# kubernetes-sigs/kube-batch

Measured on AMD Instinct MI355X. Metric: pod-node scoring evals/sec + binds/sec, 100k tasks x 10k nodes snapshot, higher is better.
Workload: dtype f64+i64

## Files before the change

### kube-batch_amd/csrc/kb_commit_sel.hip

```cpp
#include <string.h>

#include <algorithm>

#include "kb_k9.hpp"
#include "kb_repair.hpp"

#define K9S_PREP0 5u
#define K9S_PREPS 3u
#define K9S_SPIN_LIMIT (1u << 21)

__device__ __forceinline__ uint32_t k9s_ld(const uint32_t *p) { return __hip_atomic_load(p, __ATOMIC_ACQUIRE, __HIP_MEMORY_SCOPE_WORKGROUP); }
__device__ __forceinline__ void k9s_st(uint32_t *p, uint32_t v) { __hip_atomic_store(p, v, __ATOMIC_RELEASE, __HIP_MEMORY_SCOPE_WORKGROUP); }
__device__ __forceinline__ bool k9s_wait(K9Sync &Y, const uint32_t *p, uint32_t need, uint32_t nap = 1u) {
  uint32_t spins = 0;
  for (;;) {
    if (k9s_ld(p) >= need) return true;
    if ((++spins & 31u) == 0u) {
      if (k9s_ld(&Y.stop) | k9s_ld(&Y.err)) return k9s_ld(p) >= need;
      if (spins > K9S_SPIN_LIMIT) { k9s_st(&Y.err, 1u); return false; }
    }
    if (nap == 0u) { } else if (nap == 1u) __builtin_amdgcn_s_sleep(1); else if (nap <= 4u) __builtin_amdgcn_s_sleep(4); else __builtin_amdgcn_s_sleep(16);
  }
}

__global__ void __launch_bounds__(K9_THREADS) k_commit_select(const K9KernArgs ka) {
  KbCommitArgs a = ka.hot;
  {
    const unsigned char __attribute__((address_space(4))) *kp = (const unsigned char __attribute__((address_space(4))) *)__builtin_amdgcn_kernarg_segment_ptr();
    a.dev = (const KbDev *)(kp + offsetof(K9KernArgs, dev));
    a.round = (const KbRound *)(kp + offsetof(K9KernArgs, round));
  }
  extern __shared__ __align__(16) unsigned char k9_smem[];
  if ((blockIdx.x & 7u) != 0u && a.round->lists_ready != nullptr) {
    const uint32_t row = blockIdx.x - 1u - blockIdx.x / 8u;
    if (row < a.n_mrows && !KB_CHAIN_BROKEN(*a.round)) kb_repair_row<K9_THREADS>(*a.dev, *a.round, k9_smem, row, threadIdx.x);
    return;
  }
  if (k9_preamble(a)) return;
  const uint32_t tid = threadIdx.x, lane = tid & 63, wave = tid >> 6;
  const uint32_t S = a.n_mrows, W = a.n_rows;
  const K9Layout lo = k9_layout(W, S, a.L, a.NP, a.R, true);
  unsigned char *k9_base_ = k9_smem;
  K9_LDS_VIEWS(lo)
  (void)shp; (void)S; (void)dk; (void)ckey; (void)cpos;
  K9Sel &X = *reinterpret_cast<K9Sel *>(k9_smem + lo.sel);
  K9Sync &Y = X.sync;
  const unsigned long long t_start = wall_clock64();
#ifdef KB_K9_TRACE
  unsigned long long t_stage[2] = {0ull, 0ull};
  const bool staged = k9_prologue(a, lo, k9_smem, tid, 0u, t_stage);
#else
  const bool staged = k9_prologue(a, lo, k9_smem, tid, 0u);
#endif
  if (!staged) {
    if (tid == 0) k9_publish_skipped(a);
// ... 18 lines not shown
  __syncthreads();
  if (tid < W) {
    uint32_t w = tid >> 5, mword = X.brk[w] & (0xFFFFFFFFu >> (31u - (tid & 31u)));
    while (mword == 0u) { w--; mword = X.brk[w]; }
    const uint32_t p = 32u * w + (31u - (uint32_t)__clz((int)mword));
    if ((tid - p) % K9_SEL_MAXRUN == 0u) atomicOr(&X.stm[tid >> 5], 1u << (tid & 31));
  }
  __syncthreads();
  if (tid < W && ((X.stm[tid >> 5] >> (tid & 31)) & 1u)) {
    uint32_t kidx = (uint32_t)__popc(X.stm[tid >> 5] & ((1u << (tid & 31)) - 1u));
    for (uint32_t w = 0; w < (tid >> 5); w++) kidx += (uint32_t)__popc(X.stm[w]);
    X.runs[kidx] = (uint16_t)tid;
  }
  __syncthreads();
  uint32_t K = 0;
  for (uint32_t w = 0; w < 8; w++) K += (uint32_t)__popc(X.stm[w]);
  {
    uint4 rr = make_uint4(0u, 0u, 0u, 0u);
    uint32_t i0c = 0u;
    uint32_t rlen = 0u;
    if (tid < K) { i0c = X.runs[tid]; rr = rinfo[i0c]; rlen = ((tid + 1u < K) ? (uint32_t)X.runs[tid + 1u] : W) - i0c; }
    __syncthreads();
    if (tid < K) rinfo[tid] = make_uint4(i0c | (rlen << 16), rr.y, rr.z, rr.w);
    __syncthreads();
  }

#ifdef KB_K9_TRACE
  uint32_t tacc[10] = {0, 0, 0, 0, 0, 0, 0, 0, 0, 0};
  const unsigned long long t_tab = wall_clock64();
  tacc[1] = (uint32_t)(t_stage[0] - t_start); tacc[9] = (uint32_t)(t_stage[1] - t_stage[0]); tacc[2] = (uint32_t)(t_tab - t_stage[1]);
  unsigned long long tlast = __builtin_readcyclecounter();
#define K9S_TR(k, t0) do { if (lane == 0) atomicAdd(&X.tr[k], (uint32_t)(__builtin_readcyclecounter() - (t0))); } while (0)
#define K9S_NOW() __builtin_readcyclecounter()
#else
#define K9S_TR(k, t0) do { (void)(t0); } while (0)
#define K9S_NOW() 0ull
#endif
#ifndef KB_K9_NAP_PREP
#define KB_K9_NAP_PREP 1u
#endif
  constexpr uint32_t nap_prep = KB_K9_NAP_PREP, nap_dk = 1u;
#if !defined(KB_K9_PRIO) || KB_K9_PRIO
#define K9S_SETPRIO(p) __builtin_amdgcn_s_setprio(p)
#else
#define K9S_SETPRIO(p) do { } while (0)
#endif
  const unsigned long long lt = (1ull << lane) - 1ull;
  gptrd gi, gr;
  { const KbDev &d = *a.dev; gi = (gptrd)d.idle; gr = (gptrd)d.rel; }
#define K9S_RUN_HEADER_OF(ri_)                                                                                         \
  const uint32_t hx_ = (uint32_t)__builtin_amdgcn_readfirstlane((int)(ri_).x);                                          \
  const uint32_t i0 = hx_ & 0xFFFFu, r = hx_ >> 16, s = (uint32_t)__builtin_amdgcn_readfirstlane((int)(ri_).y);          \
  const uint32_t fl0 = (uint32_t)__builtin_amdgcn_readfirstlane((int)(ri_).z), km0 = (uint32_t)__builtin_amdgcn_readfirstlane((int)(ri_).w); \
  const bool plain0 = (fl0 & 1u) && (km0 == 0u || (fl0 & 4u));                                                         \
  const bool sel_run = !a.backfill && plain0 && r >= 2u && a.whole;             \
  (void)sel_run; (void)i0;
#define K9S_RUN_SHAPE(kk)                                                                                              \
  const K9Shape sh = shapes[s];                                                                                        \
  const double *si = sinit + (size_t)s * RS;                                                                           \
  const double *rres = rowres + ((kk) % K9S_PREPS) * (uint32_t)a.R;    \
  const double *rqv = plain0 ? si : rres + 2;                                             \
  (void)rqv; (void)rres;
#define K9S_RUN_HEADER(kk)                                                                                             \
  const uint4 ri_ = rinfo[(kk)];                                                                                       \
  K9S_RUN_HEADER_OF(ri_)                                                                                               \
  K9S_RUN_SHAPE(kk)

  if (wave == 0) {
    K9S_SETPRIO(3);
    uint32_t nd = 0, n_dirty_rows = 0, n_runs = 0, n_slow = 0, i_end = 0, reason_end = KB_REASON_DONE;
    uint32_t prev_nd0 = 0, prev_pc = 0;
    bool prev_chg = true;
    bool prev_all = false;
    uint4 hd_next = rinfo[0];
    for (uint32_t k = 0; k < K; k++) {
      uint32_t lane_i = tid;
      asm volatile("" : "+v"(lane_i));
      const uint4 hd = hd_next;
      if (k + 1u < K) hd_next = rinfo[k + 1u];
      K9S_RUN_HEADER_OF(hd)
      K9_STAMP(3);
      {
        uint32_t spins = 0;
        bool ok = true;
        for (;;) {
          const uint32_t *wp = (lane_i == 0u) ? (prev_all ? &Y.seq_spec : &Y.seq_cand) : (prev_chg ? &Y.seq_dk[(lane_i - 1u) & 3u] : &Y.seq_early[(lane_i - 1u) & 3u]);
          const uint32_t v = (lane_i < 5u) ? k9s_ld(wp) : 0xFFFFFFFFu;
          if (__ballot(v < k + 1u) == 0ull) break;
          if ((++spins & 31u) == 0u && (k9s_ld(&Y.err) || spins > K9S_SPIN_LIMIT)) { k9s_st(&Y.err, 1u); ok = false; break; }
          __builtin_amdgcn_s_sleep(1);
        }
        if (!ok) { reason_end = KB_REASON_INTERNAL; i_end = i0; break; }
      }
      if (prev_all && lane_i == 0) k9s_st(&Y.seq_cand, k + 1u);
      const uint32_t ncand = Y.ncand_at[k & 3u];
      const K9Sel::Cand &CD = X.cand[k & 1u];
      const uint32_t *dk = X.dkb[k & 1u];
      uint32_t *chg = Y.chg[k & 1u];
      uint32_t ck = CD.ckey[lane_i], k1 = CD.ck1[lane_i], ckind = CD.ckind[lane_i];
      const uint32_t cpos = CD.cpos[lane_i];
      uint32_t m = (lane_i < 4u) ? (prev_chg ? Y.mdk[k & 1u][lane_i] : Y.mdko[k & 1u][lane_i]) : 0u;
      if (!prev_chg && lane_i >= 4u && lane_i - 4u < prev_pc) m = dk[prev_nd0 + lane_i - 4u];
      if (lane_i < 10u) chg[lane_i] = 0u;
      K9_STAMP(0);
      if (lane_i >= ncand) { ck = 0u; k1 = 0u; ckind = 0u; }
      m = wave_max_u32(m);
      uint32_t pc = 0, j = 0, reason = KB_REASON_DONE, n_dirty = 0, sc_dirty = 0;
      bool chg_any = false;
      bool run_done = false;
      if (!a.backfill && plain0) {
        const uint32_t cmin = (ncand == r) ? rl32(ck, r - 1u) : 0u;
        const unsigned long long deeper = __ballot(lane_i + 1u < r && ckind == 0u && k1 > cmin);
        if (ncand == r && m < cmin && !deeper) {
          const unsigned long long pipes = __ballot(lane_i < r && ckind != 0u);
          const uint32_t n_take = pipes ? (uint32_t)__ffsll((unsigned long long)pipes) : r;
          if (pipes) reason = KB_REASON_PIPELINED;
          if (lane_i < n_take) {
            const uint32_t n = nmaskbits - (ck & nmaskbits);
            ldec[i0 + lane_i] = (unsigned long long)n | ((unsigned long long)ckind << 32);
            atomicOr(&bitmap[n >> 5], 1u << (n & 31));
            if (km0) {
              const double *rqv = sinit + (size_t)s * RS;
              const uint32_t rnm = CD.crnm[lane_i];
              atomicOr(&chg[(nd + lane_i) >> 5], 1u << ((nd + lane_i) & 31));
              const bool has_map = ckind ? (rnm >> 31) : (rnm & 0x7FFFFFFFu);
              if (has_map)
                for (uint32_t mm = km0, dd = 0; mm; mm >>= 1, dd++)
                  if (mm & 1u) k9_sc_sub(ckind ? gr : gi, a.NP, dd, n, rqv[dd]);
            }
          }
          if (km0) { sc_dirty = 1; chg_any = true; }
          pc = n_take; j = n_take;
          run_done = true;
          if (lane_i == 0 && r >= 2u) atomicAdd(&X.stat[0], 1u);
          K9_STAMP(8);
        }
      }
      if (!run_done) {
      K9S_RUN_SHAPE(k)
      uint32_t rnm = 0;
      if (lane_i < ncand) rnm = CD.crnm[lane_i];
      double res0 = sh.init0, res1 = sh.init1;
      if (!plain0) { res0 = rres[0]; res1 = rres[1]; }
      uint32_t d0 = 0u, d1 = 0u, d2 = 0u, d3 = 0u;
      bool have_d = false;
#define K9S_LOAD_D() do { if (!have_d) { d0 = (lane_i < nd) ? dk[lane_i] : 0u; d1 = (lane_i + 64 < nd) ? dk[lane_i + 64] : 0u; d2 = (lane_i + 128 < nd) ? dk[lane_i + 128] : 0u; \
                                        d3 = (lane_i + 192 < nd) ? dk[lane_i + 192] : 0u; have_d = true; } } while (0)
      bool sel_done = false;
      if (sel_run) {
        K9S_LOAD_D();
        bool pooled = false;
        while (j < r) {
          const uint32_t rem = r - j;
          const uint32_t fidx = pc + rem - 1u;
          uint32_t thr = max(fidx < ncand ? rl32(ck, fidx) : 0u, 1u);
          const uint32_t kc = lane_i < pc ? k1 : (lane_i < ncand ? ck : 0u);
          bool isc, is0, is1, is2, is3;
          unsigned long long bc, b0, b1, b2, b3;
          uint32_t nc_, n0_, n1_, n2_, n3_, nC;
          for (uint32_t again = 0;; again++) {
            isc = kc >= thr; is0 = d0 >= thr; is1 = d1 >= thr; is2 = d2 >= thr; is3 = d3 >= thr;
            bc = __ballot(isc); b0 = __ballot(is0);
            nc_ = (uint32_t)__popcll(bc); n0_ = (uint32_t)__popcll(b0);
            b1 = 0ull; b2 = 0ull; b3 = 0ull; n1_ = 0u; n2_ = 0u; n3_ = 0u;
            if (nd > 64u) { b1 = __ballot(is1); n1_ = (uint32_t)__popcll(b1); }
            if (nd > 128u) { b2 = __ballot(is2); b3 = __ballot(is3); n2_ = (uint32_t)__popcll(b2); n3_ = (uint32_t)__popcll(b3); }
            nC = nc_ + n0_ + n1_ + n2_ + n3_;
            if (nC <= 32u || again) break;
            uint32_t lm = max(max(max(d0, d1), max(d2, d3)), kc);
            for (uint32_t t = 0; t < 5u; t++) {
              const uint32_t mx = wave_max_u32(lm);
              if (mx == 0u) break;
              thr = mx;
              if (lm == mx) lm = 0u;
            }
          }
          if (nC == 0u) { reason = KB_REASON_NO_FEASIBLE; break; }
          {
            const uint32_t p_c = (uint32_t)__popcll(bc & lt), p_0 = nc_ + (uint32_t)__popcll(b0 & lt);
            if (isc) { X.c_slot[p_c] = (nd + lane_i) | (lane_i >= pc ? 0x80000000u : 0u); X.c_key[p_c] = kc; }
            if (is0) { X.c_slot[p_0] = lane_i; X.c_key[p_0] = d0; }
// ... 236 lines not shown
          if (bf_bulk) {
            const uint32_t left1 = (uint32_t)(rl64(cur8, F_CLS_LEFT) >> 32);
            bulk = 1u + min(r - j - 1u, left1);
            if (bulk > 1u) {
              if (lane_i == F_NZC) { double z = u2d(cur8); for (uint32_t t = 1; t < bulk; t++) z += sh.nzc; cur8 = d2u(z); }
              else if (lane_i == F_NZM) { double z = u2d(cur8); for (uint32_t t = 1; t < bulk; t++) z += sh.nzm; cur8 = d2u(z); }
              else if (lane_i == F_CLS_LEFT) cur8 -= ((unsigned long long)(bulk - 1u) << 32);
            }
          }
          if (lane_i < K9_NF) st[lane_i] = cur8;
          if (lane_i < bulk) ldec[i0 + j + lane_i] = (unsigned long long)n | ((unsigned long long)kind << 32);
          j += bulk - 1u;
          n_dirty += bulk - 1u;
          K9_WAVE_FENCE();
          const bool more = j + 1u < r && !kind;
          const uint32_t adjm1 = (!kind && has_map) ? km0 : 0u;
          uint32_t nk = 0u;
          if (more) nk = k9_eval_v(a, sh, k9_load(st), scs, gi, gr, si, adjm1, 1.0, rqv, nb, nmaskbits);
          if (km0 && has_map) {
            if (sc_lane && ((km0 >> sd) & 1u)) k9_sc_sub(kind ? gr : gi, a.NP, sd, n, rqv[sd]);
            sc_dirty = 1;
          }
          if (more) {
            if (lane_i == L) {
              if (is_new) k1 = nk;
              else if (wsel == 0) d0 = nk; else if (wsel == 1) d1 = nk; else if (wsel == 2) d2 = nk; else d3 = nk;
            }
            m = wave_max_u32(max(max(max(d0, d1), max(d2, d3)), (lane_i < pc) ? k1 : 0u));
          }
          n_dirty++;
        }
        if (kind) { j++; reason = KB_REASON_PIPELINED; break; }
      }
      }
      if (sc_dirty) __threadfence();
      const uint32_t i_next = i0 + j;
      uint32_t stop = (reason != KB_REASON_DONE || k + 1u >= K) ? 1u : 0u;
      if (!stop && a.has_aff && !a.backfill && i_next != 0u) {
        const uint32_t fln = (uint32_t)__builtin_amdgcn_readfirstlane((int)hd_next.z);
        if (fln & 2u) { reason = KB_REASON_RENORM; stop = 1u; }
      }
      if (pc) { const uint32_t cp = rl32(cpos, pc - 1u); if (lane_i == 0) cursor[s] = cp + 1u; }
      prev_nd0 = nd; prev_pc = pc; prev_all = pc == ncand;
      K9_WAVE_FENCE();
      prev_chg = chg_any;
      nd += pc; n_dirty_rows += n_dirty; n_runs += 1u; n_slow += plain0 ? 0u : 1u;
      i_end = i_next; reason_end = reason;
      if (lane_i == 0) {
        Y.nd_at[(k + 1u) & 3u] = nd;
        Y.spec_ok[(k + 1u) & 3u] = prev_all ? 1u : 0u;
        if (stop) k9s_st(&Y.stop, 1u);
        k9s_st(&Y.seq_done, k + 1u);
      }
      if (stop) break;
    }
#ifdef KB_K9_TRACE
    tacc[4] = (uint32_t)(wall_clock64() - t_tab);
#endif
    if (lane == 0) {
      if (k9s_ld(&Y.err)) reason_end = KB_REASON_INTERNAL;
      k9s_st(&Y.stop, 1u);
      H.i = i_end; H.nd = nd; H.reason = reason_end; H.n_dirty_rows = n_dirty_rows; H.n_runs = n_runs; H.n_slow = n_slow;
    }
  } else if (wave <= 4u) {
    K9S_SETPRIO(2);
    const uint32_t t = tid - 64u;
    for (uint32_t q = 0; q < K; q++) {
      K9S_RUN_HEADER(q)
      uint32_t *dko = X.dkb[q & 1u];
      uint32_t key = 0u, nd_early = 0u;
      const unsigned long long tw0 = K9S_NOW();
      if (q >= 1u) {
        if (!k9s_wait(Y, &Y.seq_done, q - 1u, nap_dk) || !k9s_wait(Y, &Y.seq_cand, q, nap_dk) || k9s_ld(&Y.stop)) break;
        nd_early = Y.nd_at[(q - 1u) & 3u] + Y.ncand_at[(q - 1u) & 3u];
        if (t < nd_early) {
          const K9St vs = k9_load(slots + (size_t)t * K9_NF);
          const K9Sc scp = k9_sc_preload(sh.active >> 2, gi, gr, a.NP, vs.node);
          key = k9_eval_v(a, sh, vs, scp, gi, gr, si, 0u, 0.0, si, nb, nmaskbits);
          dko[t] = key;
        }
        const uint32_t wmo = wave_max_u32(t < Y.nd_at[(q - 1u) & 3u] ? key : 0u);
        if (lane == 0) Y.mdko[q & 1u][wave - 1u] = wmo;
      }
      if (lane == 0) k9s_st(&Y.seq_early[wave - 1u], q + 1u);
      if (wave == 1u) K9S_TR(3, tw0);
      const unsigned long long tw1 = K9S_NOW();
      if (!k9s_wait(Y, &Y.seq_done, q, nap_dk) || k9s_ld(&Y.stop)) break;
      if (wave == 1u) K9S_TR(2, tw1);
      const uint32_t nd = Y.nd_at[q & 3u];
      if (t < nd && (t >= nd_early || ((Y.chg[(q - 1u) & 1u][t >> 5] >> (t & 31)) & 1u))) {
        const K9St vs = k9_load(slots + (size_t)t * K9_NF);
        const K9Sc scp = k9_sc_preload(sh.active >> 2, gi, gr, a.NP, vs.node);
        key = k9_eval_v(a, sh, vs, scp, gi, gr, si, 0u, 0.0, si, nb, nmaskbits);
      }
      if (t >= nd) key = 0u;
      if (t < K9_MAXSLOTS) dko[t] = key;
      const uint32_t wm = wave_max_u32(key);
      if (lane == 0) { Y.mdk[q & 1u][wave - 1u] = wm; k9s_st(&Y.seq_dk[wave - 1u], q + 1u); }
    }
  } else if (wave < K9S_PREP0 + K9S_PREPS) {
    typedef const unsigned long long __attribute__((address_space(1))) *gptr8;
    typedef const uint32_t __attribute__((address_space(1))) *gptr4;
    gptr8 g8[10];
    gptr8 gports;
    gptr4 gcls, gmaxp, gpodc, gnm;
    {
      const KbDev &d = *a.dev;
      g8[0] = (gptr8)reinterpret_cast<const unsigned long long *>(d.idle); g8[1] = (gptr8)reinterpret_cast<const unsigned long long *>(d.idle + d.NP);
      g8[2] = (gptr8)reinterpret_cast<const unsigned long long *>(d.rel); g8[3] = (gptr8)reinterpret_cast<const unsigned long long *>(d.rel + d.NP);
      g8[4] = (gptr8)reinterpret_cast<const unsigned long long *>(d.inv_acpu); g8[5] = (gptr8)reinterpret_cast<const unsigned long long *>(d.inv_amem);
      g8[6] = (gptr8)reinterpret_cast<const unsigned long long *>(d.acpu); g8[7] = (gptr8)reinterpret_cast<const unsigned long long *>(d.amem);
      g8[8] = (gptr8)reinterpret_cast<const unsigned long long *>(d.nzc); g8[9] = (gptr8)reinterpret_cast<const unsigned long long *>(d.nzm);
      gports = (gptr8)d.ports;
      gcls = (gptr4)d.ncls; gmaxp = (gptr4)reinterpret_cast<const uint32_t *>(d.maxpods); gpodc = (gptr4)reinterpret_cast<const uint32_t *>(d.podcnt); gnm = (gptr4)d.nmask;
    }
    K9Prep &P = X.prep[wave - K9S_PREP0];
    for (uint32_t m = wave - K9S_PREP0; m < K; m += K9S_PREPS) {
      K9S_RUN_HEADER(m)
      const uint32_t r1 = m >= 1u ? (uint32_t)X.runs[m] - (uint32_t)X.runs[m - 1u] : 0u, r2 = m >= 2u ? (uint32_t)X.runs[m - 1u] - (uint32_t)X.runs[m - 2u] : 0u;
      uint32_t want = r + r1 + r2, need = m >= 2u ? m - 2u : 0u;
      if (want > 64u) { want = r + r1; need = m >= 1u ? m - 1u : 0u; }
      const unsigned long long tp0 = K9S_NOW();
      if (!k9s_wait(Y, &Y.seq_done, need, nap_prep) || k9s_ld(&Y.stop)) break;
      K9S_TR(1, tp0);
      uint32_t nf = 0;
      {
        uint32_t e_ = cursor[s];
        while (nf < want) {
          const uint32_t pos_ = e_ + lane;
          const uint32_t kk_ = (pos_ < Lp) ? lists[s * Lp + pos_] : 0u;
          const bool nz_ = kk_ != 0u;
          const uint32_t nn_ = nmaskbits - (kk_ & nmaskbits);
          const bool cl_ = nz_ && !((bitmap[(nz_ ? nn_ : 0u) >> 5] >> (nn_ & 31)) & 1u);
          const unsigned long long zeros_ = __ballot(!nz_);
          const uint32_t fz_ = zeros_ ? (uint32_t)__ffsll((unsigned long long)zeros_) - 1u : 64u;
          const unsigned long long clean_ = __ballot(cl_ && lane < fz_);
          const uint32_t rank_ = (uint32_t)__popcll(clean_ & lt);
          if (((clean_ >> lane) & 1ull) && nf + rank_ < want) { P.ckey[nf + rank_] = kk_; P.cpos[nf + rank_] = pos_; }
          nf = min(want, nf + (uint32_t)__popcll(clean_));
          if (fz_ < 64u || e_ + 64u >= Lp) break;
          e_ += 64u;
        }
        K9_WAVE_FENCE();
      }
      const uint32_t key = (lane < nf) ? P.ckey[lane] : 0u, mypos = (lane < nf) ? P.cpos[lane] : 0u;
      const uint32_t n = nmaskbits - (key & nmaskbits);
      unsigned long long raw[11] = {0, 0, 0, 0, 0, 0, 0, 0, 0, 0, 0};
      uint32_t rcls = 0, rmaxp = 0, rpodc = 0, rnm = 0;
      if (lane < nf) {
#pragma unroll
        for (int f = 0; f < 10; f++) raw[f] = g8[f][n];
        raw[F_PORTS] = gports ? gports[n] : 0ull;
        rcls = gcls[n]; rmaxp = gmaxp[n]; rpodc = gpodc[n]; rnm = gnm[n];
      }
      if (!plain0 && lane == 63) {
        const KbDev &d_ = *a.dev;
// ... 22 lines not shown
        v.ports = raw[F_PORTS] | sh.want;
        v.cls = rcls; v.node = lane < nf ? n : 0u; v.left = (int)rmaxp - (int)rpodc - 1;
        const uint32_t adjm = (!kind && (rnm & 0x7FFFFFFFu)) ? km0 : 0u;
        if (lane < nf) {
          k1 = k9_eval_v(a, sh, v, scn, gi, gr, si, adjm, 1.0, rqv, nb, nmaskbits);
        }
      }
      K9Sel::Cand &CD = X.cand[m & 1u];
      auto settle = [&](bool ahead) {
        uint32_t nd0 = Y.nd_at[m & 3u];
        bool keep = lane < nf && !((bitmap[n >> 5] >> (n & 31)) & 1u);
        if (ahead) {
          const K9Sel::Cand &CP = X.cand[(m - 1u) & 1u];
          const uint32_t ncp = Y.ncand_at[(m - 1u) & 3u];
          nd0 = Y.nd_at[(m - 1u) & 3u] + ncp;
          for (uint32_t i = 0; i < ncp; i++) keep = keep && (nmaskbits - (CP.ckey[i] & nmaskbits)) != n;
        }
        const unsigned long long kb = __ballot(keep);
        const uint32_t rho = (uint32_t)__popcll(kb & lt);
        const uint32_t ncand = min((uint32_t)__popcll(kb), r);
        if (keep && rho < r) {
          unsigned long long *st = slots + (size_t)(nd0 + rho) * K9_NF;
          st[F_IDLE0] = d2u(v.idle0); st[F_IDLE1] = d2u(v.idle1); st[F_REL0] = d2u(v.rel0); st[F_REL1] = d2u(v.rel1);
          st[F_INVAC] = raw[F_INVAC]; st[F_INVAM] = raw[F_INVAM]; st[F_AC] = d2u(v.ac); st[F_AM] = d2u(v.am);
          st[F_NZC] = d2u(v.nzc); st[F_NZM] = d2u(v.nzm); st[F_PORTS] = v.ports;
          st[F_CLS_LEFT] = (unsigned long long)rcls | ((unsigned long long)(uint32_t)v.left << 32);
          st[F_NODE_NMASK] = (unsigned long long)n | ((unsigned long long)rnm << 32);
          CD.ckey[rho] = key; CD.cpos[rho] = mypos;
          CD.ckind[rho] = kind; CD.ck1[rho] = k1; CD.crnm[rho] = rnm;
        }
        if (lane == 0) Y.ncand_at[m & 3u] = ncand;
      };
      if (m >= 1u) {
        if (!k9s_wait(Y, &Y.seq_cand, m, nap_prep) || k9s_ld(&Y.stop)) break;
        settle(true);
        if (lane == 0) k9s_st(&Y.seq_spec, m + 1u);
      }
      const unsigned long long tp1 = K9S_NOW();
      if (!k9s_wait(Y, &Y.seq_done, m, nap_prep) || k9s_ld(&Y.stop)) break;
      K9S_TR(0, tp1);
      if (m == 0u || !Y.spec_ok[m & 3u]) {
        settle(false);
        if (lane == 0) k9s_st(&Y.seq_cand, m + 1u);
      }
    }
  }
#ifdef KB_K9_TRACE
  if (tid == 0) {
    unsigned long long *tw = reinterpret_cast<unsigned long long *>(a.result);
    tw[5] = (unsigned long long)tacc[0] | ((unsigned long long)tacc[1] << 32);
    tw[6] = (unsigned long long)tacc[2] | ((unsigned long long)tacc[3] << 32);
    tw[7] = (unsigned long long)tacc[4] | ((unsigned long long)tacc[5] << 32);
    tw[13] = (unsigned long long)tacc[6] | ((unsigned long long)tacc[7] << 32);
    tw[14] = (unsigned long long)tacc[8] | ((unsigned long long)tacc[9] << 32);
  }
#endif
  __syncthreads();
#ifdef KB_K9_TRACE
  if (tid == 0) {
    unsigned long long *tw = reinterpret_cast<unsigned long long *>(a.result);
    tw[4] = (unsigned long long)X.tr[0] | ((unsigned long long)X.tr[1] << 32);
    tw[15] = (unsigned long long)X.tr[2] | ((unsigned long long)X.tr[3] << 32);
  }
#endif
  k9_epilogue(a, lo, k9_smem, tid, t_start, X.stat[0] | (X.stat[1] << 16), X.stat[2] | (X.stat[3] << 16), true, job_of_my_row);
}

void kb_launch_commit_sel(const KbDev &d, const KbRound &r, void *stream) {
  if (r.n_rows == 0) return;
  static bool lds_set[64] = {};
  k9_allow_full_lds(reinterpret_cast<const void *>(k_commit_select), lds_set);
  size_t sh = k9_layout(r.n_rows, r.n_mrows, r.L, d.NP, d.R, true).total;
  if (r.lists_ready != nullptr) sh = std::max(sh, kb_repair_lds_bytes(d.NP, K9_THREADS));
  K9KernArgs ka;
  k9_fill_args(ka, d, r);
  static_assert(KB_REPAIR_THREADS == K9_THREADS, "the repair workgroups of a fused launch are workgroups of this kernel");
  uint32_t grid = KB_WARM_GRID;
  if (r.lists_ready != nullptr) grid = std::max<uint32_t>(grid, r.n_mrows + (r.n_mrows - 1u) / 7u + 1u);
  static const bool solo = [] { const char *v = getenv("KB_PROFILE_SOLO_COMMIT"); return v && v[0] == '1'; }();
  if (solo && r.lists_ready == nullptr) grid = 1u;
  hipLaunchKernelGGL(k_commit_select, dim3(grid), dim3(K9_THREADS), sh, (hipStream_t)stream, ka);
}
```

### kube-batch_amd/csrc/kb_engine.cpp

```cpp
#include "kb_engine_int.hpp"

thread_local std::string g_create_err;

namespace kbe {

void ensure_window_buffers(kb_engine *e, uint32_t rows) {
  if (rows <= e->win_cap) return;
  if (!e->b_desc.p) e->b_desc.alloc(sizeof(KbRowDesc) * 2 * KB_K5_MAX_WINDOW);
  e->h_rows.resize(rows);
  e->h_slot.resize(rows);
  e->h_decnode.resize(rows);
  e->h_deckind.resize(rows);
  e->win_cap = rows;
}
void ensure_ip_scratch(kb_engine *e, size_t rows) {
  if (!e->hs.has_interpod) return;
  const size_t NP = e->dev.NP;
  if (e->b_ip_scnt.bytes < sizeof(long long) * rows * NP) {
    e->b_ip_scnt.alloc(sizeof(long long) * rows * NP);
    e->b_ip_shist.alloc(sizeof(int32_t) * rows * NP);
  }
  e->dev.ip_scratch_cnt = e->b_ip_scnt.as<long long>();
  e->dev.ip_scratch_hist = e->b_ip_shist.as<int32_t>();
}
// ... 151 lines not shown
void kb_engine_destroy(kb_engine *e) {
  if (!e) return;
  if (getenv("KB_K5_STATS"))
    fprintf(stderr, "[kb K5] rounds on the run kernel %llu, on the selection kernel %llu, last dirty share %.3f\n",
            (unsigned long long)e->rounds_run, (unsigned long long)e->rounds_sel, e->dirty_share);
  if (getenv("KB_K5_STATS") && e->rounds_sel)
    fprintf(stderr, "[kb select] runs of >= 2 rows: all picks clean first placements %llu, committed by shots %llu (shots cut short by a table's end %llu; shots %llu)\n",
            (unsigned long long)e->sel_stat[0], (unsigned long long)e->sel_stat[1], (unsigned long long)e->sel_stat[2], (unsigned long long)e->sel_stat[3]);
  if (getenv("KB_K5_STATS"))
    fprintf(stderr, "[kb K5] rounds %llu, rows %llu, dirty slots %llu, dirty-won rows %llu, runs %llu, runs with a row-specific Resreq %llu (%llu)\n",
            (unsigned long long)e->stats.rounds, (unsigned long long)e->stats.decisions, (unsigned long long)e->k5_slots,
            (unsigned long long)e->stats.row_fallbacks, (unsigned long long)e->k5_walks, (unsigned long long)e->k5_rescans,
            (unsigned long long)e->k5_demand);
  if (getenv("KB_K5_STATS")) fprintf(stderr, "[kb overlap] rounds with candidate lists built beside the predecessor's commit %llu, lists that never arrived %llu; repair launches: %.3f ms from their start to the tag seen\n",
                                     (unsigned long long)e->overlapped_rounds, (unsigned long long)e->overlap_faults, e->tl_repair_tag);
  if (getenv("KB_K5_STATS"))
    fprintf(stderr, "[kb host] ms over the engine's life: reset %.2f, allocate up to its first launch %.2f, speculation breaks (answer -> re-planned launch) %.2f, "
            "closing reductions %.2f, waiting for rounds %.2f, backfill up to its first launch %.2f\n", e->tl_reset, e->tl_begin, e->tl_break, e->tl_finish, e->tl_wait, e->tl_backfill);
  if (getenv("KB_K5_STATS"))
    fprintf(stderr, "[kb host] of the start: order machine %.2f, first probe %.2f, first plan %.2f; of the breaks: probe launch + absorb %.2f, waiting for the probe %.2f, re-plan %.2f\n",
            e->tl_begin_parts[0], e->tl_begin_parts[1], e->tl_begin_parts[2], e->tl_break_parts[0], e->tl_break_parts[1], e->tl_break_parts[2]);
  if (getenv("KB_K5_STATS")) fprintf(stderr, "[kb probe] %llu probes, %llu shapes marked dead by them\n", (unsigned long long)e->probes, (unsigned long long)e->probe_deaths);
  if (getenv("KB_K5_STATS") && e->k5_trace[0] > 0) {
    static const char *ph[10] = {"barrier 1 (wave 0's wait)", "evaluate: candidates (wave 0)", "barrier 2", "rows", "prepare the next run",
                                "rows, of runs with scalar dimensions", "runs with scalar dimensions (count)", "evaluate, of runs with scalar dimensions",
                                "dirty-winner entries (count)", "loop top"};
    static const char *ph_sel[10] = {"wave 0 waits for candidates + dirty keys", "staging: lists, descriptors (10 ns units, not clocks)", "run tables (10 ns units)", "rows: serial loop, tail, publish", "wave 0's loop (10 ns units)",
                                    "selection: entries + first rank", "selection: deep passes", "selection: picks + AddTask", "selection: all picks clean", "shape tables (10 ns units)"};
    const double runs = (double)(e->k5_walks ? e->k5_walks : 1);
    for (int k = 0; k < 10; k++) fprintf(stderr, "[kb K5 trace] %-32s %14.0f clocks  (%.0f per run)\n", e->rounds_sel > e->rounds_run ? ph_sel[k] : ph[k], e->k5_trace[k], e->k5_trace[k] / runs);
    static const char *ph_role[4] = {"prep waves wait for their run's turn (sum of 3)", "prep waves wait for the walk's turn (sum of 3)", "wave 1 waits for the previous run", "wave 1 evaluates + publishes"};
    if (e->rounds_sel > e->rounds_run) for (int k = 10; k < 14; k++) fprintf(stderr, "[kb K5 trace] %-32s %14.0f clocks  (%.0f per run)\n", ph_role[k - 10], e->k5_trace[k], e->k5_trace[k] / runs);
  }
  (void)hipSetDevice(e->device);
  delete e;
}

int kb_get_binds(kb_engine *e, uint32_t *task_node_out) {
  if (!e) return KB_E_INVALID;
  return guarded(e, [&]() {
    if (!e->loaded) throw EngineError(KB_E_STATE, "no session loaded");
    quiesce(e);
    HIP_OK(hipMemcpy(task_node_out, e->b_tbind.p, sizeof(uint32_t) * e->hs.T, hipMemcpyDeviceToHost));
    uint64_t nb = 0;
    for (uint32_t t = 0; t < e->hs.T; t++) nb += task_node_out[t] != KB_NONE;
    e->stats.binds = nb;
  });
}

int kb_get_task_state(kb_engine *e, uint8_t *status_out, uint32_t *node_out) {
  if (!e) return KB_E_INVALID;
  return guarded(e, [&]() {
    if (!e->loaded) throw EngineError(KB_E_STATE, "no session loaded");
    quiesce(e);
    if (status_out) HIP_OK(hipMemcpy(status_out, e->b_tstatus.p, e->hs.T, hipMemcpyDeviceToHost));
    if (node_out) HIP_OK(hipMemcpy(node_out, e->b_tnode.p, sizeof(uint32_t) * e->hs.T, hipMemcpyDeviceToHost));
  });
}

int kb_get_node_state(kb_engine *e, double *idle, double *releasing, int64_t *nz_cpu, int64_t *nz_mem, int32_t *pod_cnt) {
  if (!e) return KB_E_INVALID;
  return guarded(e, [&]() {
    if (!e->loaded) throw EngineError(KB_E_STATE, "no session loaded");
    quiesce(e);
    const uint32_t N = e->hs.N, NP = e->dev.NP;
    const int R = e->hs.R;
// ... 44 lines not shown
```

### kube-batch_amd/csrc/kb_engine_int.hpp

```cpp
#pragma once
#include <hip/hip_runtime.h>

#include <sched.h>

#include <chrono>
#include <cstdio>
#include <cstdlib>
#include <functional>
#include <map>
#include <memory>
#include <string>
#include <unordered_map>
#include <vector>

#include "../../include/kb_engine.h"
#include "kb_device.h"
#include "kb_host.hpp"
#include "kb_waterfill.hpp"
#include "kb_preempt.hpp"

using namespace kb;

#define HIP_OK(expr)                                                                                      \
  do {                                                                                                    \
// ... 128 lines not shown
    HIP_OK(hipEventCreate(&a));
    HIP_OK(hipEventCreate(&b));
  }
  void destroy() {
    if (a) (void)hipEventDestroy(a);
    if (b) (void)hipEventDestroy(b);
    a = b = nullptr;
  }
};

}
using namespace kbe;

struct MgState;
void mg_free(MgState *m);
void mg_reset(MgState *m);

struct kb_engine {
  std::string err;
  int device = 0;
  uint32_t window = 256, commit_batch = 0, flags = 0;
  Policy pol;
  hipStream_t stream = nullptr, own_stream = nullptr;
  bool loaded = false;
  bool tainted = false;
  HostSession hs;
  KbDev dev{};
  kb_stats stats{};
  uint64_t round_no = 0;

  DevBuf b_idle, b_rel, b_nzc, b_nzm, b_podcnt, b_acpu, b_amem, b_maxpods, b_ncls, b_nmask, b_invac, b_invam;
  uint64_t k5_walks = 0, k5_rescans = 0, k5_demand = 0, k5_slots = 0;
  double k5_trace[14] = {0, 0, 0, 0, 0, 0, 0, 0, 0, 0, 0, 0, 0, 0};
  double tl_repair_tag = 0;
  uint32_t eff_window = 0;
  int commit_kernel = KB_COMMIT_SELECT, commit_pin = -1;
  double dirty_share = 0.0;
  uint64_t rounds_run = 0, rounds_sel = 0;
  uint64_t sel_stat[4] = {0, 0, 0, 0};
  uint32_t shape_cap = KB_K5_MAX_SHAPES;
  std::vector<uint32_t> plan_stamp;
  uint32_t plan_epoch = 0;
  const double *t_fit = nullptr;
  bool idle_below_eps = false;
  DevBuf b_tfit;
  DevBuf b_tinit, b_tres, b_tnzc, b_tnzm, b_tcls, b_tactive, b_tresmask, b_tjob, b_tstatus, b_tnode, b_tbind, b_tcounted, b_jallocated, b_compat, b_crows, b_aff, b_affcls;
  DevBuf p_idle, p_rel, p_nzc, p_nzm, p_podcnt, p_tstatus, p_tnode, p_tcounted, p_ports, p_nmask;
  DevBuf b_ip_cdom, b_ip_ccnt, b_ip_ctot, b_ip_tinc, b_ip_tforbid, b_ip_treq, b_ip_tself, b_ip_tsubj, b_ip_tchk, b_ip_pdom, b_ip_pbound, b_ip_punb, b_ip_tcinc,
      b_ip_tsig, b_ip_sigw, b_ip_z, b_ip_scnt, b_ip_shist, p_ip_ccnt, p_ip_ctot, p_ip_punb, p_ip_z;
  DevBuf b_ports, b_twant, b_tconf;
  DevBuf b_ports_x, b_twant_x, b_tconf_x, p_ports_x;
  DevBuf b_jbegin, b_jmin, b_jqueue, b_total, b_deserved, b_desmask, b_jalloc, b_jshare, b_qalloc, b_qshare, b_jready;
  uint32_t total_mask = 0;
  DevBuf b_desc;
  Pinned<unsigned long long> h_listkeys;
  Pinned<unsigned char> h_evict;
  DevBuf b_scatter;
  Pinned<unsigned long long> h_scatter;
  DevBuf b_sscore, b_smask, b_xslot, b_xorder, b_xchunks;
  std::vector<uint32_t> h_xorder;
  std::vector<KbXChunk> h_xchunks;
  size_t xs_cap = 0, xslot_cap = 0;
  DevBuf b_mrows, b_same, b_score, b_maskw, b_keys;
  hipStream_t stream_b = nullptr;
  DevBuf b_score2, b_maskw2, b_stale, b_ready, b_task_rows, b_lready;
  bool fuse_repair = true;
// ... 390 lines not shown
```

### kube-batch_amd/csrc/kb_k9.hpp

```cpp
#pragma once
#include <hip/hip_runtime.h>
#include <stddef.h>
#include <stdint.h>
#include <stdlib.h>

#include "kb_device.h"
#include "kb_eval.hpp"
#include "kb_warm.hpp"

#define K9_THREADS 512
#define K9_MAXRUN 64
#define K9_SEL_MAXRUN 32
#define K9_MAXSLOTS 256
#define K9_NF 13
enum { F_IDLE0 = 0, F_IDLE1, F_REL0, F_REL1, F_INVAC, F_INVAM, F_AC, F_AM, F_NZC, F_NZM, F_PORTS, F_CLS_LEFT, F_NODE_NMASK };

struct K9Shape {
  double init0, init1, nzc, nzm;
  unsigned long long conf, want;
  uint32_t cls, active, crow, pad;
};

struct K9Hdr {
  uint32_t i, nd, reason, stop;
  uint32_t ncand, n_dirty_rows, n_runs, n_slow;
  uint32_t cur_s, cur_r, cur_fl, cur_km;
};

struct K9Prep {
  uint32_t ckey[64], cpos[64];
};
struct K9Sync {
  uint32_t seq_done;
  uint32_t seq_cand;
  uint32_t seq_dk[4];
  uint32_t seq_early[4];
  uint32_t seq_spec;
  uint32_t spec_ok[4];
  uint32_t stop, err;
  uint32_t nd_at[4];
  uint32_t ncand_at[4];
  uint32_t mdk[2][4];
  uint32_t mdko[2][4];
  uint32_t chg[2][10];
};
struct K9Sel {
  K9Sync sync;
  K9Prep prep[3];
  uint16_t runs[KB_K5_MAX_ROWS];
  uint32_t brk[8], stm[8];
  struct Cand { uint32_t ckey[64], cpos[64], ckind[64], ck1[64], crnm[64]; } cand[2];
  uint32_t dkb[2][K9_MAXSLOTS];
  uint32_t c_slot[64], c_sorted[64];
  alignas(16) uint32_t c_key[64];
  alignas(16) uint32_t e_eff[64];
  uint32_t e_key[64];
  uint32_t pool[K9_MAXSLOTS + 64];
  uint32_t tr[4];
  uint32_t stat[4];
};

struct K9Layout {
  uint32_t slots, rowres, sinit, shapes, desc, rinfo, dec, hdr, dk, ckey, cpos, cursor, shp, lists, bitmap, sel, total;
  uint32_t Lp, RS;
};
__host__ __device__ inline K9Layout k9_layout(uint32_t n_rows, uint32_t n_shapes, uint32_t L, uint32_t NP, int R, bool sel = false) {
  K9Layout o;
  o.RS = R > 2 ? (uint32_t)(R - 2) : 0u;
  o.Lp = L;
  uint32_t off = 0;
  o.slots = off;  off += (n_rows + K9_MAXRUN) * K9_NF * 8u;
  o.rowres = off; off += 3u * (uint32_t)R * 8u;
  o.sinit = off;  off += n_shapes * o.RS * 8u;
  o.shapes = off; off += n_shapes * (uint32_t)sizeof(K9Shape);
  o.desc = off;   off += n_rows * (uint32_t)sizeof(KbRowDesc);
  off = (off + 15u) & ~15u;
  o.rinfo = off;  off += n_rows * 16u;
  o.dec = off;    off += n_rows * 8u;
  o.hdr = off;    off += (uint32_t)sizeof(K9Hdr);
  o.dk = off;     off += K9_MAXSLOTS * 4u;
  o.ckey = off;   off += K9_MAXRUN * 4u;
  o.cpos = off;   off += K9_MAXRUN * 4u;
  o.cursor = off; off += n_shapes * 4u;
  o.shp = off;    off += n_shapes * 4u;
  o.lists = off;  off += n_shapes * o.Lp * 4u;
  o.bitmap = off; off += (NP / 32u) * 4u;
  off = (off + 15u) & ~15u;
  o.sel = 0;
  if (sel) { o.sel = off; off += (uint32_t)sizeof(K9Sel); }
  o.total = (off + 15u) & ~15u;
  return o;
// ... 429 lines not shown
```

### kube-batch_amd/csrc/kb_rounds.cpp

```cpp
#include "kb_engine_int.hpp"

namespace kbe {

KbRound make_round(kb_engine *e, uint32_t n_rows, uint32_t n_mrows, uint32_t L, int fit_mode, bool backfill, uint32_t buf) {
  KbRound r{};
  r.rows = e->b_win.as<uint32_t>();
  r.shape_slot = e->b_win.as<uint32_t>() + KB_K5_MAX_WINDOW;
  r.n_rows = n_rows;
  r.desc = e->b_desc.as<KbRowDesc>() + (size_t)buf * KB_K5_MAX_WINDOW;
  r.trace = nullptr;
  r.cap = std::max<uint32_t>(64, ((n_rows + 63) / 64) * 64);
  r.mrows = e->b_win.as<uint32_t>() + 2 * KB_K5_MAX_WINDOW;
  r.mrow_task0 = 0;
  r.same_prev = nullptr;
  r.n_mrows = n_mrows;
  r.fit_mode = fit_mode;
  r.score = e->b_score.as<uint16_t>();
  r.maskw = e->b_maskw.as<uint32_t>();
  r.keys = e->b_keys.as<unsigned long long>();
  r.L = L;
  r.dec = e->b_out.as<unsigned long long>() + KB_OUT_HDR;
  r.result = e->b_out.as<uint32_t>();
  r.host_out = nullptr;
  r.seq = 0;
  r.backfill = backfill ? 1 : 0;
  r.batch = 0;
  r.gather = 0;
  r.delta = nullptr;
  r.own_row0 = r.own_row1 = 0;
  return r;
}

uint32_t assign_shapes(kb_engine *e, uint32_t n, const uint32_t *rows) {
  HostSession &hs = e->hs;
  if (!rows) rows = e->h_rows.data();
  if (e->shape_stamp.size() != hs.n_row_shapes) {
    e->shape_stamp.assign(hs.n_row_shapes, 0);
    e->shape_slot_of.assign(hs.n_row_shapes, 0);
    e->stamp = 0;
  }
  e->stamp++;
  uint32_t ns = 0;
  for (uint32_t i = 0; i < n; i++) {
// ... 528 lines not shown
```

Baseline: 21.26 billion.

## Wake sleeping waves on hand-off, look three runs ahead, publish before writing decisions

Adds s_wakeup calls after every sequence-counter publish, and changes the shared wait loop to poll relaxed with an acquire fence and a longer s_sleep, so waiting waves resume sooner after a hand-off. Prep waves may now prepare candidates three runs ahead when the combined run length fits in 64. The serial walk wave now publishes seq_done before writing its decision words and stats, which takes that store off the critical hand-off path. It also adds optional trace counters. The costs are extra wakeup instructions and a lower spin limit, and the later decision write depends on readers not needing ldec before the next step.

```diff
diff --git a/kube-batch_amd/csrc/kb_commit_sel.hip b/kube-batch_amd/csrc/kb_commit_sel.hip
--- a/kube-batch_amd/csrc/kb_commit_sel.hip
+++ b/kube-batch_amd/csrc/kb_commit_sel.hip
@@ -11,16 +11,61 @@
 
 __device__ __forceinline__ uint32_t k9s_ld(const uint32_t *p) { return __hip_atomic_load(p, __ATOMIC_ACQUIRE, __HIP_MEMORY_SCOPE_WORKGROUP); }
 __device__ __forceinline__ void k9s_st(uint32_t *p, uint32_t v) { __hip_atomic_store(p, v, __ATOMIC_RELEASE, __HIP_MEMORY_SCOPE_WORKGROUP); }
-__device__ __forceinline__ bool k9s_wait(K9Sync &Y, const uint32_t *p, uint32_t need, uint32_t nap = 1u) {
+#ifndef KB_K9_WAKE
+#define KB_K9_WAKE 1
+#endif
+#if KB_K9_WAKE
+#define K9S_WAKE() asm volatile("s_wakeup" ::: "memory")
+#define K9S_WAIT_LIMIT (1u << 19)
+#else
+#define K9S_WAKE() ((void)0)
+#define K9S_WAIT_LIMIT K9S_SPIN_LIMIT
+#endif
+#ifdef KB_K9_TRACE
+#define K9S_TA(tsi, bk) , &X, (tsi), (bk)
+#else
+#define K9S_TA(tsi, bk)
+#endif
+__device__ __forceinline__ bool k9s_wait(K9Sync &Y, const uint32_t *p, uint32_t need, uint32_t nap = 1u, bool ping = false
+#ifdef KB_K9_TRACE
+                                         , K9Sel *xt = nullptr, uint32_t tsi = 0u, uint32_t bk = 0u
+#endif
+                                         ) {
   uint32_t spins = 0;
   for (;;) {
+#if KB_K9_WAKE
+    const uint32_t v = __hip_atomic_load(p, __ATOMIC_RELAXED, __HIP_MEMORY_SCOPE_WORKGROUP), st = __hip_atomic_load(&Y.stop, __ATOMIC_RELAXED, __HIP_MEMORY_SCOPE_WORKGROUP);
+    __builtin_amdgcn_fence(__ATOMIC_ACQUIRE, "workgroup");
+    if (v >= need) break;
+    if (st) return k9s_ld(p) >= need;
+    if ((++spins & 31u) == 0u) {
+      if (k9s_ld(&Y.err)) return false;
+      if (spins > K9S_WAIT_LIMIT) { k9s_st(&Y.err, 1u); K9S_WAKE(); return false; }
+    }
+    if (ping && spins == 1u) K9S_WAKE();
+    (void)nap;
+    __builtin_amdgcn_s_sleep(8);
+#else
+#ifdef KB_K9_TRACE
+    if (k9s_ld(p) >= need) break;
+#else
     if (k9s_ld(p) >= need) return true;
+#endif
     if ((++spins & 31u) == 0u) {
       if (k9s_ld(&Y.stop) | k9s_ld(&Y.err)) return k9s_ld(p) >= need;
       if (spins > K9S_SPIN_LIMIT) { k9s_st(&Y.err, 1u); return false; }
     }
+    (void)ping;
     if (nap == 0u) { } else if (nap == 1u) __builtin_amdgcn_s_sleep(1); else if (nap <= 4u) __builtin_amdgcn_s_sleep(4); else __builtin_amdgcn_s_sleep(16);
-  }
+#endif
+  }
+#ifdef KB_K9_TRACE
+  if (xt != nullptr && spins != 0u && (threadIdx.x & 63u) == 0u) {
+    atomicAdd(&xt->trx[bk], (uint32_t)__builtin_readcyclecounter() - xt->ts[tsi]);
+    atomicAdd(&xt->trx[bk + 1u], 1u);
+  }
+#endif
+  return true;
 }
 
 __global__ void __launch_bounds__(K9_THREADS) k_commit_select(const K9KernArgs ka) {
@@ -105,14 +150,29 @@
   unsigned long long tlast = __builtin_readcyclecounter();
 #define K9S_TR(k, t0) do { if (lane == 0) atomicAdd(&X.tr[k], (uint32_t)(__builtin_readcyclecounter() - (t0))); } while (0)
 #define K9S_NOW() __builtin_readcyclecounter()
+#define K9X_ADD(k, v) do { if (lane == 0) atomicAdd(&X.trx[k], (uint32_t)(v)); } while (0)
+#define K9X_STAMP(k) do { const unsigned long long now_ = __builtin_readcyclecounter(); K9X_ADD(k, now_ - tlast); K9X_ADD((k) + 1, 1u); tlast = now_; } while (0)
+#define K9X_TS(i) do { if (lane == 0) X.ts[i] = (uint32_t)__builtin_readcyclecounter(); } while (0)
+  if (tid < KB_TRX_WORDS) X.trx[tid] = 0u;
+  if (tid < 12) X.ts[tid] = 0u;
+  __syncthreads();
 #else
 #define K9S_TR(k, t0) do { (void)(t0); } while (0)
 #define K9S_NOW() 0ull
+#define K9X_ADD(k, v) ((void)0)
+#define K9X_STAMP(k) ((void)0)
+#define K9X_TS(i) ((void)0)
 #endif
 #ifndef KB_K9_NAP_PREP
 #define KB_K9_NAP_PREP 1u
 #endif
   constexpr uint32_t nap_prep = KB_K9_NAP_PREP, nap_dk = 1u;
+#ifndef KB_K9_AHEAD3
+#define KB_K9_AHEAD3 1
+#endif
+#ifndef KB_K9_PUBFIRST
+#define KB_K9_PUBFIRST 1
+#endif
 #if !defined(KB_K9_PRIO) || KB_K9_PRIO
 #define K9S_SETPRIO(p) __builtin_amdgcn_s_setprio(p)
 #else
@@ -156,16 +216,44 @@
       {
         uint32_t spins = 0;
         bool ok = true;
+#ifdef KB_K9_TRACE
+        unsigned long long behind_last = 0ull;
+#endif
+        K9S_WAKE();
         for (;;) {
           const uint32_t *wp = (lane_i == 0u) ? (prev_all ? &Y.seq_spec : &Y.seq_cand) : (prev_chg ? &Y.seq_dk[(lane_i - 1u) & 3u] : &Y.seq_early[(lane_i - 1u) & 3u]);
           const uint32_t v = (lane_i < 5u) ? k9s_ld(wp) : 0xFFFFFFFFu;
-          if (__ballot(v < k + 1u) == 0ull) break;
-          if ((++spins & 31u) == 0u && (k9s_ld(&Y.err) || spins > K9S_SPIN_LIMIT)) { k9s_st(&Y.err, 1u); ok = false; break; }
+          const unsigned long long behind = __ballot(v < k + 1u);
+          if (behind == 0ull) break;
+#ifdef KB_K9_TRACE
+          behind_last = behind;
+#endif
+          if ((++spins & 31u) == 0u && (k9s_ld(&Y.err) || spins > K9S_SPIN_LIMIT)) { k9s_st(&Y.err, 1u); K9S_WAKE(); ok = false; break; }
+#if KB_K9_WAKE
+          if (spins == 1u) K9S_WAKE();
+#endif
           __builtin_amdgcn_s_sleep(1);
         }
         if (!ok) { reason_end = KB_REASON_INTERNAL; i_end = i0; break; }
-      }
+#ifdef KB_K9_TRACE
+        {
+          const uint32_t now32 = (uint32_t)__builtin_readcyclecounter();
+          const uint32_t cls = spins == 0u ? 3u : ((behind_last & 1ull) ? ((behind_last & 0x1Eull) ? 2u : 0u) : 1u);
+          K9X_ADD(2u * cls, now32 - (uint32_t)tlast); K9X_ADD(2u * cls + 1u, 1u);
+          if (spins) {
+            const uint32_t tsi = (lane_i == 0u) ? (prev_all ? 10u : 9u) : ((prev_chg ? 5u : 1u) + ((lane_i - 1u) & 3u));
+            uint32_t d = (lane_i < 5u && ((behind_last >> lane_i) & 1ull)) ? now32 - X.ts[tsi] : 0xFFFFFFFFu;
+            d = ~wave_max_u32(~d);
+            K9X_ADD(cls == 1u ? 16u : 18u, d); K9X_ADD(cls == 1u ? 17u : 19u, 1u);
+          }
+        }
+#endif
+      }
+      if (prev_all) K9X_TS(9);
       if (prev_all && lane_i == 0) k9s_st(&Y.seq_cand, k + 1u);
+#if KB_K9_WAKE
+      if (prev_all) K9S_WAKE();
+#endif
       const uint32_t ncand = Y.ncand_at[k & 3u];
       const K9Sel::Cand &CD = X.cand[k & 1u];
       const uint32_t *dk = X.dkb[k & 1u];
@@ -190,7 +278,9 @@
           if (pipes) reason = KB_REASON_PIPELINED;
           if (lane_i < n_take) {
             const uint32_t n = nmaskbits - (ck & nmaskbits);
+#if !KB_K9_PUBFIRST
             ldec[i0 + lane_i] = (unsigned long long)n | ((unsigned long long)ckind << 32);
+#endif
             atomicOr(&bitmap[n >> 5], 1u << (n & 31));
             if (km0) {
               const double *rqv = sinit + (size_t)s * RS;
@@ -205,7 +295,9 @@
           if (km0) { sc_dirty = 1; chg_any = true; }
           pc = n_take; j = n_take;
           run_done = true;
+#if !KB_K9_PUBFIRST
           if (lane_i == 0 && r >= 2u) atomicAdd(&X.stat[0], 1u);
+#endif
           K9_STAMP(8);
         }
       }
@@ -220,6 +312,7 @@
 #define K9S_LOAD_D() do { if (!have_d) { d0 = (lane_i < nd) ? dk[lane_i] : 0u; d1 = (lane_i + 64 < nd) ? dk[lane_i + 64] : 0u; d2 = (lane_i + 128 < nd) ? dk[lane_i + 128] : 0u; \
                                         d3 = (lane_i + 192 < nd) ? dk[lane_i + 192] : 0u; have_d = true; } } while (0)
       bool sel_done = false;
+      K9X_STAMP(8);
       if (sel_run) {
         K9S_LOAD_D();
         bool pooled = false;
@@ -522,6 +615,9 @@
         }
         if (kind) { j++; reason = KB_REASON_PIPELINED; break; }
       }
+#ifdef KB_K9_TRACE
+      if (!sel_done) { if (r == 1u) K9X_STAMP(10); else K9X_STAMP(12); }
+#endif
       }
       if (sc_dirty) __threadfence();
       const uint32_t i_next = i0 + j;
@@ -536,12 +632,20 @@
       prev_chg = chg_any;
       nd += pc; n_dirty_rows += n_dirty; n_runs += 1u; n_slow += plain0 ? 0u : 1u;
       i_end = i_next; reason_end = reason;
+      K9X_TS(0);
       if (lane_i == 0) {
         Y.nd_at[(k + 1u) & 3u] = nd;
         Y.spec_ok[(k + 1u) & 3u] = prev_all ? 1u : 0u;
         if (stop) k9s_st(&Y.stop, 1u);
         k9s_st(&Y.seq_done, k + 1u);
       }
+      K9S_WAKE();
+#if KB_K9_PUBFIRST
+      if (run_done) {
+        if (lane_i < pc) ldec[i0 + lane_i] = (unsigned long long)(nmaskbits - (ck & nmaskbits)) | ((unsigned long long)ckind << 32);
+        if (lane_i == 0 && r >= 2u) atomicAdd(&X.stat[0], 1u);
+      }
+#endif
       if (stop) break;
     }
 #ifdef KB_K9_TRACE
@@ -561,7 +665,15 @@
       uint32_t key = 0u, nd_early = 0u;
       const unsigned long long tw0 = K9S_NOW();
       if (q >= 1u) {
+#ifdef KB_K9_TRACE
+        const bool w_a = k9s_wait(Y, &Y.seq_done, q - 1u, nap_dk, false K9S_TA(0u, 14u));
+        if (wave == 1u) K9X_ADD(24, K9S_NOW() - tw0);
+        const unsigned long long tw_b = K9S_NOW();
+        if (!w_a || !k9s_wait(Y, &Y.seq_cand, q, nap_dk, false K9S_TA(9u, 28u)) || k9s_ld(&Y.stop)) break;
+        if (wave == 1u) K9X_ADD(25, K9S_NOW() - tw_b);
+#else
         if (!k9s_wait(Y, &Y.seq_done, q - 1u, nap_dk) || !k9s_wait(Y, &Y.seq_cand, q, nap_dk) || k9s_ld(&Y.stop)) break;
+#endif
         nd_early = Y.nd_at[(q - 1u) & 3u] + Y.ncand_at[(q - 1u) & 3u];
         if (t < nd_early) {
           const K9St vs = k9_load(slots + (size_t)t * K9_NF);
@@ -572,11 +684,14 @@
         const uint32_t wmo = wave_max_u32(t < Y.nd_at[(q - 1u) & 3u] ? key : 0u);
         if (lane == 0) Y.mdko[q & 1u][wave - 1u] = wmo;
       }
+      K9X_TS(wave);
       if (lane == 0) k9s_st(&Y.seq_early[wave - 1u], q + 1u);
       if (wave == 1u) K9S_TR(3, tw0);
       const unsigned long long tw1 = K9S_NOW();
-      if (!k9s_wait(Y, &Y.seq_done, q, nap_dk) || k9s_ld(&Y.stop)) break;
+      if (!k9s_wait(Y, &Y.seq_done, q, nap_dk, false K9S_TA(0u, 14u)) || k9s_ld(&Y.stop)) break;
       if (wave == 1u) K9S_TR(2, tw1);
+      const unsigned long long tw2 = K9S_NOW();
+      (void)tw2;
       const uint32_t nd = Y.nd_at[q & 3u];
       if (t < nd && (t >= nd_early || ((Y.chg[(q - 1u) & 1u][t >> 5] >> (t & 31)) & 1u))) {
         const K9St vs = k9_load(slots + (size_t)t * K9_NF);
@@ -586,7 +701,11 @@
       if (t >= nd) key = 0u;
       if (t < K9_MAXSLOTS) dko[t] = key;
       const uint32_t wm = wave_max_u32(key);
+      K9X_TS(4u + wave);
       if (lane == 0) { Y.mdk[q & 1u][wave - 1u] = wm; k9s_st(&Y.seq_dk[wave - 1u], q + 1u); }
+#ifdef KB_K9_TRACE
+      if (wave == 1u) { K9X_ADD(26, K9S_NOW() - tw2); K9X_ADD(27, K9S_NOW() - tw0); }
+#endif
     }
   } else if (wave < K9S_PREP0 + K9S_PREPS) {
     typedef const unsigned long long __attribute__((address_space(1))) *gptr8;
@@ -610,8 +729,14 @@
       const uint32_t r1 = m >= 1u ? (uint32_t)X.runs[m] - (uint32_t)X.runs[m - 1u] : 0u, r2 = m >= 2u ? (uint32_t)X.runs[m - 1u] - (uint32_t)X.runs[m - 2u] : 0u;
       uint32_t want = r + r1 + r2, need = m >= 2u ? m - 2u : 0u;
       if (want > 64u) { want = r + r1; need = m >= 1u ? m - 1u : 0u; }
+#if KB_K9_AHEAD3
+      else if (m >= 3u && plain0) {
+        const uint32_t r3 = (uint32_t)X.runs[m - 2u] - (uint32_t)X.runs[m - 3u];
+        if (want + r3 <= 64u) { want += r3; need = m - 3u; }
+      }
+#endif
       const unsigned long long tp0 = K9S_NOW();
-      if (!k9s_wait(Y, &Y.seq_done, need, nap_prep) || k9s_ld(&Y.stop)) break;
+      if (!k9s_wait(Y, &Y.seq_done, need, nap_prep, true K9S_TA(0u, 20u)) || k9s_ld(&Y.stop)) break;
       K9S_TR(1, tp0);
       uint32_t nf = 0;
       {
@@ -700,17 +825,25 @@
         if (lane == 0) Y.ncand_at[m & 3u] = ncand;
       };
       if (m >= 1u) {
+        const unsigned long long tp2 = K9S_NOW();
+        (void)tp2;
         if (!k9s_wait(Y, &Y.seq_cand, m, nap_prep) || k9s_ld(&Y.stop)) break;
+        K9X_ADD(23, K9S_NOW() - tp2);
         settle(true);
+        K9X_TS(10);
         if (lane == 0) k9s_st(&Y.seq_spec, m + 1u);
+        K9S_WAKE();
       }
       const unsigned long long tp1 = K9S_NOW();
-      if (!k9s_wait(Y, &Y.seq_done, m, nap_prep) || k9s_ld(&Y.stop)) break;
+      if (!k9s_wait(Y, &Y.seq_done, m, nap_prep, true K9S_TA(0u, 20u)) || k9s_ld(&Y.stop)) break;
       K9S_TR(0, tp1);
       if (m == 0u || !Y.spec_ok[m & 3u]) {
         settle(false);
+        K9X_TS(9);
         if (lane == 0) k9s_st(&Y.seq_cand, m + 1u);
-      }
+        K9S_WAKE();
+      }
+      K9X_ADD(22, K9S_NOW() - tp0);
     }
   }
 #ifdef KB_K9_TRACE
@@ -730,6 +863,7 @@
     tw[4] = (unsigned long long)X.tr[0] | ((unsigned long long)X.tr[1] << 32);
     tw[15] = (unsigned long long)X.tr[2] | ((unsigned long long)X.tr[3] << 32);
   }
+  if (tid < KB_TRX_WORDS && a.trace != nullptr) atomicAdd(&a.trace[tid], (unsigned long long)X.trx[tid]);
 #endif
   k9_epilogue(a, lo, k9_smem, tid, t_start, X.stat[0] | (X.stat[1] << 16), X.stat[2] | (X.stat[3] << 16), true, job_of_my_row);
 }
diff --git a/kube-batch_amd/csrc/kb_engine.cpp b/kube-batch_amd/csrc/kb_engine.cpp
--- a/kube-batch_amd/csrc/kb_engine.cpp
+++ b/kube-batch_amd/csrc/kb_engine.cpp
@@ -207,6 +207,28 @@
     static const char *ph_role[4] = {"prep waves wait for their run's turn (sum of 3)", "prep waves wait for the walk's turn (sum of 3)", "wave 1 waits for the previous run", "wave 1 evaluates + publishes"};
     if (e->rounds_sel > e->rounds_run) for (int k = 10; k < 14; k++) fprintf(stderr, "[kb K5 trace] %-32s %14.0f clocks  (%.0f per run)\n", ph_role[k - 10], e->k5_trace[k], e->k5_trace[k] / runs);
   }
+#ifdef KB_K9_TRACE
+  if (getenv("KB_K5_STATS") && e->b_trx.p != nullptr && e->rounds_sel > e->rounds_run) {
+    unsigned long long x[KB_TRX_WORDS] = {};
+    (void)hipSetDevice(e->device);
+    (void)hipDeviceSynchronize();
+    if (hipMemcpy(x, e->b_trx.p, sizeof(x), hipMemcpyDeviceToHost) == hipSuccess) {
+      const double runs = (double)(e->k5_walks ? e->k5_walks : 1);
+      static const char *w0[7] = {"wave 0's wait ended by the candidates' word (lane 0)", "wave 0's wait ended by a dirty-key word (lanes 1-4)", "wave 0's wait, both behind at the last look",
+                                  "wave 0 did not wait (poll + loads)", "slow paths' set-up (shape, candidates' other fields)", "serial loop, single rows", "serial loop, other runs"};
+      for (int k = 0; k < 7; k++)
+        fprintf(stderr, "[kb K5 trace+] %-56s %14llu clocks in %9llu runs (%.0f each, %.0f per run of the round)\n", w0[k], x[2 * k], x[2 * k + 1], (double)x[2 * k] / (double)(x[2 * k + 1] ? x[2 * k + 1] : 1), (double)x[2 * k] / runs);
+      static const char *ho[5] = {"hand-off seq_done -> waves 1..4", "hand-off seq_early / seq_dk -> wave 0", "hand-off seq_spec / seq_cand -> wave 0", "hand-off seq_done -> a prep wave", "hand-off seq_cand -> waves 1..4"};
+      static const int hoi[5] = {14, 16, 18, 20, 28};
+      for (int k = 0; k < 5; k++)
+        fprintf(stderr, "[kb K5 trace+] %-56s %14llu clocks in %9llu waits that slept (%.0f each)\n", ho[k], x[hoi[k]], x[hoi[k] + 1], (double)x[hoi[k]] / (double)(x[hoi[k] + 1] ? x[hoi[k] + 1] : 1));
+      const double prep_busy = (double)x[22] - e->k5_trace[10] - e->k5_trace[11] - (double)x[23];
+      fprintf(stderr, "[kb K5 trace+] prep waves: iterations %llu clocks (sum of 3), wait for seq_cand %llu, busy without their three waits %.0f (%.0f per run)\n", x[22], x[23], prep_busy, prep_busy / runs);
+      fprintf(stderr, "[kb K5 trace+] wave 1: iterations %llu clocks (%.0f per run); early phase: waits for seq_done %llu + seq_cand %llu, busy %.0f (%.0f per run); final evaluation + publish %llu (%.0f per run)\n",
+              x[27], (double)x[27] / runs, x[24], x[25], e->k5_trace[13] - (double)x[24] - (double)x[25], (e->k5_trace[13] - (double)x[24] - (double)x[25]) / runs, x[26], (double)x[26] / runs);
+    }
+  }
+#endif
   (void)hipSetDevice(e->device);
   delete e;
 }
diff --git a/kube-batch_amd/csrc/kb_engine_int.hpp b/kube-batch_amd/csrc/kb_engine_int.hpp
--- a/kube-batch_amd/csrc/kb_engine_int.hpp
+++ b/kube-batch_amd/csrc/kb_engine_int.hpp
@@ -184,6 +184,10 @@
   DevBuf b_idle, b_rel, b_nzc, b_nzm, b_podcnt, b_acpu, b_amem, b_maxpods, b_ncls, b_nmask, b_invac, b_invam;
   uint64_t k5_walks = 0, k5_rescans = 0, k5_demand = 0, k5_slots = 0;
   double k5_trace[14] = {0, 0, 0, 0, 0, 0, 0, 0, 0, 0, 0, 0, 0, 0};
+#ifdef KB_K9_TRACE
+#define KB_TRX_WORDS 48u
+  DevBuf b_trx;
+#endif
   double tl_repair_tag = 0;
   uint32_t eff_window = 0;
   int commit_kernel = KB_COMMIT_SELECT, commit_pin = -1;
diff --git a/kube-batch_amd/csrc/kb_k9.hpp b/kube-batch_amd/csrc/kb_k9.hpp
--- a/kube-batch_amd/csrc/kb_k9.hpp
+++ b/kube-batch_amd/csrc/kb_k9.hpp
@@ -44,6 +44,9 @@
   uint32_t mdko[2][4];
   uint32_t chg[2][10];
 };
+#ifdef KB_K9_TRACE
+#define KB_TRX_WORDS 48u
+#endif
 struct K9Sel {
   K9Sync sync;
   K9Prep prep[3];
@@ -57,6 +60,10 @@
   uint32_t e_key[64];
   uint32_t pool[K9_MAXSLOTS + 64];
   uint32_t tr[4];
+#ifdef KB_K9_TRACE
+  uint32_t trx[KB_TRX_WORDS];
+  uint32_t ts[12];
+#endif
   uint32_t stat[4];
 };
 
diff --git a/kube-batch_amd/csrc/kb_rounds.cpp b/kube-batch_amd/csrc/kb_rounds.cpp
--- a/kube-batch_amd/csrc/kb_rounds.cpp
+++ b/kube-batch_amd/csrc/kb_rounds.cpp
@@ -9,6 +9,13 @@
   r.n_rows = n_rows;
   r.desc = e->b_desc.as<KbRowDesc>() + (size_t)buf * KB_K5_MAX_WINDOW;
   r.trace = nullptr;
+#ifdef KB_K9_TRACE
+  if (e->b_trx.p == nullptr) {
+    e->b_trx.alloc(sizeof(unsigned long long) * KB_TRX_WORDS);
+    HIP_OK(hipMemsetAsync(e->b_trx.p, 0, sizeof(unsigned long long) * KB_TRX_WORDS, e->stream));
+  }
+  r.trace = e->b_trx.as<unsigned long long>();
+#endif
   r.cap = std::max<uint32_t>(64, ((n_rows + 63) / 64) * 64);
   r.mrows = e->b_win.as<uint32_t>() + 2 * KB_K5_MAX_WINDOW;
   r.mrow_task0 = 0;
```

Result: slower. 20.09 billion (median of 2 runs) (-5.5%).
